# GBATZOLIS/conditional_score_diffusion

Measured on AMD Instinct MI355X. Metric: images/sec for 1000-step PC sampling, ddpm_paired_SR3 score net of celebA_SR3_160 (BASELINE configs[1]), 160x160, higher is better.
Workload: dtype f16x3 (every operand carried as hi + lo fp16 = 22 significand bits, 3 MFMAs per product, f32 accumulate; f32-class: the per-op test tolerance is the f32 kernel's, network error 1.9e-6 vs the reference); 1 GPU; BASELINE configs[1]: celebA_SR3_160 (ddpm_paired_SR3, nf=96, ch_mult (1,1,2,2,3,3), attn 20/10/5), 1000-step PC (reverse_diffusion + langevin, snr 0.15), batch 64 per GPU, random-init weights, synthetic LR inputs; images_per_gpu=64, global_batch=64, noise=on-device Philox4x32-10, precision_mode=fp16x3

## Files before the change

conditional_score_diffusion_amd/csrc/attention.hip:

```cpp
#include "common.h"

namespace csd {

typedef float floatx16 __attribute__((ext_vector_type(16)));

#define ATT_THREADS 256
#define ATT_KT 32

template <int NCT>
__global__ __launch_bounds__(ATT_THREADS) void attention_kernel(const float* __restrict__ qkv, int ld,
                                                                float* __restrict__ out, int L,
                                                                float scale) {
  constexpr int C = NCT * 32;
  constexpr int KS = C + 4;
  extern __shared__ __attribute__((aligned(16))) float smem[];
  float* const Ks = smem;
  float* const Vs = smem + ATT_KT * KS;

  const int tid = threadIdx.x;
  const int lane = tid & 63;
  const int wave = tid >> 6;
  const int half = lane >> 5;
  const int b = blockIdx.y;
  const int q0 = blockIdx.x * 128 + wave * 32;
  const bool wave_active = q0 < L;
  const int qrow = min(q0 + (lane & 31), L - 1);
  const float* qptr = qkv + ((size_t)b * L + qrow) * ld + half * 4;
  const float* kvbase = qkv + (size_t)b * L * ld;

  floatx16 o[NCT];
#pragma unroll
  for (int n = 0; n < NCT; ++n)
#pragma unroll
    for (int r = 0; r < 16; ++r) o[n][r] = 0.f;
  float m_run = -INFINITY;
  float l_run = 0.f;

  const int ntiles = (L + ATT_KT - 1) / ATT_KT;
  for (int t = 0; t < ntiles; ++t) {
    const int key0 = t * ATT_KT;
    __syncthreads();
    for (int e = tid; e < 2 * ATT_KT * (C / 4); e += ATT_THREADS) {
      const int which = e / (ATT_KT * (C / 4));
      const int r = e - which * ATT_KT * (C / 4);
      const int key = r / (C / 4);
      const int c4 = r - key * (C / 4);
      float4 v = make_float4(0.f, 0.f, 0.f, 0.f);
      if (key0 + key < L)
        v = *reinterpret_cast<const float4*>(kvbase + (size_t)(key0 + key) * ld + (1 + which) * C + c4 * 4);
      *reinterpret_cast<float4*>((which ? Vs : Ks) + key * KS + c4 * 4) = v;
    }
    __syncthreads();
    if (!wave_active) continue;

    floatx16 s;
#pragma unroll
    for (int r = 0; r < 16; ++r) s[r] = 0.f;
    const float* krow = Ks + (lane & 31) * KS + half * 4;
#pragma unroll 4
    for (int c0 = 0; c0 < C; c0 += 8) {
      const float4 a4 = *reinterpret_cast<const float4*>(krow + c0);
      const float4 b4 = *reinterpret_cast<const float4*>(qptr + c0);
      s = __builtin_amdgcn_mfma_f32_32x32x2f32(a4.x, b4.x, s, 0, 0, 0);
      s = __builtin_amdgcn_mfma_f32_32x32x2f32(a4.y, b4.y, s, 0, 0, 0);
      s = __builtin_amdgcn_mfma_f32_32x32x2f32(a4.z, b4.z, s, 0, 0, 0);
      s = __builtin_amdgcn_mfma_f32_32x32x2f32(a4.w, b4.w, s, 0, 0, 0);
    }
    float mt = -INFINITY;
#pragma unroll
    for (int r = 0; r < 16; ++r) {
      const int key = key0 + (r & 3) + 8 * (r >> 2) + 4 * half;
      s[r] = (key < L) ? s[r] * scale : -INFINITY;
      mt = fmaxf(mt, s[r]);
    }
    mt = fmaxf(mt, __shfl_xor(mt, 32));
    const float m_new = fmaxf(m_run, mt);
    const float alpha = expf(m_run - m_new);
    float psum = 0.f;
#pragma unroll
    for (int r = 0; r < 16; ++r) {
      s[r] = expf(s[r] - m_new);
      psum += s[r];
    }
    l_run = l_run * alpha + psum;
    m_run = m_new;
#pragma unroll
    for (int r = 0; r < 16; ++r) {
      const int row = (r & 3) + 8 * (r >> 2) + 4 * half;
      const float ar = __shfl(alpha, row);
#pragma unroll
      for (int n = 0; n < NCT; ++n) o[n][r] *= ar;
    }
#pragma unroll
    for (int r = 0; r < 16; ++r) {
      const float* vrow = Vs + ((r & 3) + 8 * (r >> 2) + 4 * half) * KS + (lane & 31);
#pragma unroll
      for (int n = 0; n < NCT; ++n)
        o[n] = __builtin_amdgcn_mfma_f32_32x32x2f32(s[r], vrow[n * 32], o[n], 0, 0, 0);
    }
  }

  if (!wave_active) return;
  const float l_tot = l_run + __shfl_xor(l_run, 32);
#pragma unroll
  for (int r = 0; r < 16; ++r) {
    const int row = (r & 3) + 8 * (r >> 2) + 4 * half;
    const float lr = __shfl(l_tot, row);
    const int q = q0 + row;
    if (q < L) {
      float* dst = out + ((size_t)b * L + q) * C + (lane & 31);
#pragma unroll
      for (int n = 0; n < NCT; ++n) dst[n * 32] = o[n][r] / lr;
    }
  }
}

template <int NCT>
static int launch_att(const float* qkv, int ld, float* out, int B, int L, hipStream_t s) {
  constexpr int C = NCT * 32;
  const size_t lds = (size_t)2 * ATT_KT * (C + 4) * sizeof(float);
  auto kern = attention_kernel<NCT>;
  static bool attr_set = false;
  if (!attr_set) {
    CSD_CHECK_HIP(hipFuncSetAttribute(reinterpret_cast<const void*>(kern),
                                      hipFuncAttributeMaxDynamicSharedMemorySize, 160 * 1024));
    attr_set = true;
  }
  const float scale = 1.0f / sqrtf((float)C);
  (void)scale;
  const float ref_scale = (float)pow((double)C, -0.5);
  hipLaunchKernelGGL(kern, dim3(cdiv(L, 128), B), dim3(ATT_THREADS), lds, s, qkv, ld, out, L, ref_scale);
  CSD_LAUNCH_CHECK();
  return CSD_OK;
}

typedef _Float16 half8a __attribute__((ext_vector_type(8)));
typedef _Float16 half4a __attribute__((ext_vector_type(4)));

template <int NCT, int NS, int CS>
__global__ __launch_bounds__(ATT_THREADS) void attention16_kernel(const float* __restrict__ qkv, int ld,
                                                                  float* __restrict__ out, int L, float scale) {
  constexpr int C = NCT * 32, KSTEPS = C / 16;
  constexpr int KS = 2 * C + 16;
  constexpr int VS = 80;
  constexpr int KPL = ATT_KT * KS, VPL = C * VS;
  extern __shared__ __attribute__((aligned(16))) char smem16[];
  char* const Kp = smem16;
  char* const Vp = smem16 + NS * KPL;

  const int tid = threadIdx.x;
  const int lane = tid & 63;
  const int wave = tid >> 6;
  const int kb = lane >> 5, l32 = lane & 31;
  const int b = blockIdx.y;
  constexpr int NOT = (NCT + CS - 1) / CS;
  const int n0 = (wave % CS) * NOT;
  const int q0 = blockIdx.x * (128 / CS) + (wave / CS) * 32;
  const bool wave_active = q0 < L;
  const float* kvbase = qkv + (size_t)b * L * ld;

  half8a qh[KSTEPS], ql[NS == 2 ? KSTEPS : 1];
  {
    const float* qptr = kvbase + (size_t)min(q0 + l32, L - 1) * ld + kb * 8;
#pragma unroll
    for (int ks = 0; ks < KSTEPS; ++ks) {
      const float4 a = *reinterpret_cast<const float4*>(qptr + ks * 16);
      const float4 c = *reinterpret_cast<const float4*>(qptr + ks * 16 + 4);
      const float v[8] = {a.x * scale, a.y * scale, a.z * scale, a.w * scale, c.x * scale, c.y * scale, c.z * scale, c.w * scale};
#pragma unroll
      for (int j = 0; j < 8; ++j) {
        const _Float16 h = (_Float16)v[j];
        qh[ks][j] = h;
        if (NS == 2) ql[ks][j] = (_Float16)(v[j] - (float)h);
      }
    }
  }

  floatx16 o[NOT];
#pragma unroll
  for (int n = 0; n < NOT; ++n)
#pragma unroll
    for (int r = 0; r < 16; ++r) o[n][r] = 0.f;
  float m_run = -INFINITY, l_run = 0.f;

  constexpr int NK = NCT;
  constexpr int NVG = (2 * C + ATT_THREADS - 1) / ATT_THREADS;
  float4 prek[NK], prev[NVG][4];
  auto prefetch = [&](int key0) {
#pragma unroll
    for (int i = 0; i < NK; ++i) {
      const int e = tid + i * ATT_THREADS;
      const int key = e / (C / 4), c4 = e - key * (C / 4);
      prek[i] = key0 + key < L ? *reinterpret_cast<const float4*>(kvbase + (size_t)(key0 + key) * ld + C + c4 * 4)
                               : make_float4(0.f, 0.f, 0.f, 0.f);
    }
#pragma unroll
    for (int i = 0; i < NVG; ++i) {
      const int g = tid + i * ATT_THREADS;
      const int m = g & 7, c4 = min(g >> 3, C / 4 - 1);
#pragma unroll
      for (int u = 0; u < 4; ++u) {
        const int key = key0 + 4 * m + u;
        prev[i][u] = key < L ? *reinterpret_cast<const float4*>(kvbase + (size_t)key * ld + 2 * C + c4 * 4)
                             : make_float4(0.f, 0.f, 0.f, 0.f);
      }
    }
  };
  auto commit = [&]() {
#pragma unroll
    for (int i = 0; i < NK; ++i) {
      const int e = tid + i * ATT_THREADS;
      const int key = e / (C / 4), c4 = e - key * (C / 4);
      const float v[4] = {prek[i].x, prek[i].y, prek[i].z, prek[i].w};
      half4a hi, lo;
#pragma unroll
      for (int j = 0; j < 4; ++j) {
        hi[j] = (_Float16)v[j];
        lo[j] = (_Float16)(v[j] - (float)hi[j]);
      }
      *reinterpret_cast<half4a*>(Kp + key * KS + c4 * 8) = hi;
      if (NS == 2) *reinterpret_cast<half4a*>(Kp + KPL + key * KS + c4 * 8) = lo;
    }
#pragma unroll
    for (int i = 0; i < NVG; ++i) {
      const int g = tid + i * ATT_THREADS;
      if (g >= 2 * C) continue;
      const int m = g & 7, c4 = g >> 3;
      const int w = (4 * m) & 15;
      const int pos = ((4 * m) & 16) + 8 * ((w >> 2) & 1) + 4 * (w >> 3);
#pragma unroll
      for (int j = 0; j < 4; ++j) {
        const float v[4] = {j == 0 ? prev[i][0].x : j == 1 ? prev[i][0].y : j == 2 ? prev[i][0].z : prev[i][0].w,
                            j == 0 ? prev[i][1].x : j == 1 ? prev[i][1].y : j == 2 ? prev[i][1].z : prev[i][1].w,
                            j == 0 ? prev[i][2].x : j == 1 ? prev[i][2].y : j == 2 ? prev[i][2].z : prev[i][2].w,
                            j == 0 ? prev[i][3].x : j == 1 ? prev[i][3].y : j == 2 ? prev[i][3].z : prev[i][3].w};
        half4a hi, lo;
#pragma unroll
        for (int u = 0; u < 4; ++u) {
          hi[u] = (_Float16)v[u];
          lo[u] = (_Float16)(v[u] - (float)hi[u]);
        }
        *reinterpret_cast<half4a*>(Vp + (c4 * 4 + j) * VS + pos * 2) = hi;
        if (NS == 2) *reinterpret_cast<half4a*>(Vp + VPL + (c4 * 4 + j) * VS + pos * 2) = lo;
      }
    }
  };

  constexpr bool AHEAD = NCT <= 6;
  const int ntiles = (L + ATT_KT - 1) / ATT_KT;
  if (AHEAD) prefetch(0);
  for (int t = 0; t < ntiles; ++t) {
    const int key0 = t * ATT_KT;
    if (!AHEAD) prefetch(key0);
    __syncthreads();
    commit();
    __syncthreads();
    if (AHEAD && t + 1 < ntiles) prefetch(key0 + ATT_KT);
    if (!wave_active) continue;

    floatx16 s;
#pragma unroll
    for (int r = 0; r < 16; ++r) s[r] = 0.f;
    const char* krow = Kp + l32 * KS + kb * 16;
    half8a ah_n = *reinterpret_cast<const half8a*>(krow), al_n;
    if (NS == 2) al_n = *reinterpret_cast<const half8a*>(krow + KPL);
#pragma unroll
    for (int ks = 0; ks < KSTEPS; ++ks) {
      const half8a ah = ah_n, al = al_n;
      if (ks + 1 < KSTEPS) {
        ah_n = *reinterpret_cast<const half8a*>(krow + (ks + 1) * 32);
        if (NS == 2) al_n = *reinterpret_cast<const half8a*>(krow + KPL + (ks + 1) * 32);
      }
      if (NS == 2) {
        s = __builtin_amdgcn_mfma_f32_32x32x16_f16(al, qh[ks], s, 0, 0, 0);
        s = __builtin_amdgcn_mfma_f32_32x32x16_f16(ah, ql[ks], s, 0, 0, 0);
      }
      s = __builtin_amdgcn_mfma_f32_32x32x16_f16(ah, qh[ks], s, 0, 0, 0);
      __builtin_amdgcn_sched_barrier(0);
    }
    float mt = -INFINITY;
#pragma unroll
    for (int r = 0; r < 16; ++r) {
      const int key = key0 + (r & 3) + 8 * (r >> 2) + 4 * kb;
      s[r] = (key < L) ? s[r] : -INFINITY;
      mt = fmaxf(mt, s[r]);
    }
    mt = fmaxf(mt, __shfl_xor(mt, 32));
    const float m_new = fmaxf(m_run, mt);
    const float alpha = __expf(m_run - m_new);
    float psum = 0.f;
    half8a ph[2], pl[NS == 2 ? 2 : 1];
#pragma unroll
    for (int r = 0; r < 16; ++r) {
      const float pv = __expf(s[r] - m_new);
      psum += pv;
      const _Float16 h = (_Float16)pv;
      ph[r >> 3][r & 7] = h;
      if (NS == 2) pl[r >> 3][r & 7] = (_Float16)(pv - (float)h);
    }
    l_run = l_run * alpha + psum;
    m_run = m_new;
    if (!__all(alpha == 1.0f)) {
#pragma unroll
      for (int r = 0; r < 16; ++r) {
        const float ar = __shfl(alpha, (r & 3) + 8 * (r >> 2) + 4 * kb);
#pragma unroll
        for (int n = 0; n < NOT; ++n) o[n][r] *= ar;
      }
    }
#pragma unroll
    for (int tt = 0; tt < 2; ++tt) {
      const char* vrow = Vp + (n0 * 32 + l32) * VS + (16 * tt + 8 * kb) * 2;
      half8a vh_n = *reinterpret_cast<const half8a*>(vrow), vl_n;
      if (NS == 2) vl_n = *reinterpret_cast<const half8a*>(vrow + VPL);
#pragma unroll
      for (int n = 0; n < NOT; ++n) {
        if (CS > 1 && n0 + n >= NCT) break;
        const half8a vh = vh_n, vl = vl_n;
        if (n + 1 < NOT && (CS == 1 || n0 + n + 1 < NCT)) {
          vh_n = *reinterpret_cast<const half8a*>(vrow + (n + 1) * 32 * VS);
          if (NS == 2) vl_n = *reinterpret_cast<const half8a*>(vrow + VPL + (n + 1) * 32 * VS);
        }
        if (NS == 2) {
          o[n] = __builtin_amdgcn_mfma_f32_32x32x16_f16(pl[tt], vh, o[n], 0, 0, 0);
          o[n] = __builtin_amdgcn_mfma_f32_32x32x16_f16(ph[tt], vl, o[n], 0, 0, 0);
        }
        o[n] = __builtin_amdgcn_mfma_f32_32x32x16_f16(ph[tt], vh, o[n], 0, 0, 0);
        __builtin_amdgcn_sched_barrier(0);
      }
    }
  }

  if (!wave_active) return;
  const float l_tot = l_run + __shfl_xor(l_run, 32);
#pragma unroll
  for (int r = 0; r < 16; ++r) {
    const int row = (r & 3) + 8 * (r >> 2) + 4 * kb;
    const float lr = __shfl(l_tot, row);
    const int q = q0 + row;
    if (q < L) {
      float* dst = out + ((size_t)b * L + q) * C + n0 * 32 + l32;
#pragma unroll
      for (int n = 0; n < NOT; ++n)
        if (CS == 1 || n0 + n < NCT) dst[n * 32] = o[n][r] / lr;
    }
  }
}

template <int NCT, int NS>
static int launch_att16(const float* qkv, int ld, float* out, int B, int L, hipStream_t s) {
  constexpr int C = NCT * 32;
  const size_t lds = (size_t)NS * (ATT_KT * (2 * C + 16) + C * 80);
  constexpr int CS = NCT >= 8 ? 2 : 1;
  auto kern = attention16_kernel<NCT, NS, CS>;
  static bool attr_set = false;
  if (!attr_set) {
    CSD_CHECK_HIP(hipFuncSetAttribute(reinterpret_cast<const void*>(kern),
                                      hipFuncAttributeMaxDynamicSharedMemorySize, 160 * 1024));
    attr_set = true;
  }
  const float ref_scale = (float)pow((double)C, -0.5);
  hipLaunchKernelGGL(kern, dim3(cdiv(L, 128 / CS), B), dim3(ATT_THREADS), lds, s, qkv, ld, out, L, ref_scale);
  CSD_LAUNCH_CHECK();
  return CSD_OK;
}

int attention16_launch(const float* qkv, int ld, float* out, int B, int L, int C, int ns, hipStream_t s) {
  CSD_REQUIRE(C % 32 == 0, "attention: C=%d must be a multiple of 32", C);
  CSD_REQUIRE(L >= 1, "attention: empty sequence");
  CSD_REQUIRE(ns == 1 || ns == 2, "attention16: %d operand planes", ns);
#define CSD_ATT16_CASE(N) case N: return ns == 2 ? launch_att16<N, 2>(qkv, ld, out, B, L, s) : launch_att16<N, 1>(qkv, ld, out, B, L, s);
  switch (C / 32) {
    CSD_ATT16_CASE(1) CSD_ATT16_CASE(2) CSD_ATT16_CASE(3) CSD_ATT16_CASE(4) CSD_ATT16_CASE(6) CSD_ATT16_CASE(8) CSD_ATT16_CASE(9)
    default:
      set_error("attention: C=%d not instantiated (supported: 32,64,96,128,192,256,288)", C);
      return CSD_ERR_INVALID;
  }
#undef CSD_ATT16_CASE
}

int attention_launch(const float* qkv, int ld, float* out, int B, int L, int C, hipStream_t s) {
  CSD_REQUIRE(C % 32 == 0, "attention: C=%d must be a multiple of 32", C);
  CSD_REQUIRE(L >= 1, "attention: empty sequence");
  switch (C / 32) {
    case 1: return launch_att<1>(qkv, ld, out, B, L, s);
    case 2: return launch_att<2>(qkv, ld, out, B, L, s);
    case 3: return launch_att<3>(qkv, ld, out, B, L, s);
    case 4: return launch_att<4>(qkv, ld, out, B, L, s);
    case 6: return launch_att<6>(qkv, ld, out, B, L, s);
    case 8: return launch_att<8>(qkv, ld, out, B, L, s);
    case 9: return launch_att<9>(qkv, ld, out, B, L, s);
    default:
      set_error("attention: C=%d not instantiated (supported: 32,64,96,128,192,256,288)", C);
      return CSD_ERR_INVALID;
  }
}

}
```

Measured before the change: 1.661 images/sec.

## Use buffer loads for K/V prefetch and pin attention accumulators in AGPRs

Replaces the per-element bounds-checked global loads of K and V tiles with raw buffer loads through a buffer resource whose range ends at row L, so out-of-range keys return zero from hardware instead of via per-load compares and 64-bit address math. Offsets are precomputed once as 32-bit values, and the wave index is made uniform with readfirstlane. For wide channel counts, the output accumulators are forced into accumulation registers via inline asm constraints, with the alpha rescale done through a VGPR round trip. This lowers VGPR pressure and address arithmetic, at the cost of a 4GB offset limit (now checked at launch) and possible extra moves between register files.

```diff
diff --git a/conditional_score_diffusion_amd/csrc/attention.hip b/conditional_score_diffusion_amd/csrc/attention.hip
--- a/conditional_score_diffusion_amd/csrc/attention.hip
+++ b/conditional_score_diffusion_amd/csrc/attention.hip
@@ -136,6 +136,8 @@
 
 typedef _Float16 half8a __attribute__((ext_vector_type(8)));
 typedef _Float16 half4a __attribute__((ext_vector_type(4)));
+typedef float att_f4 __attribute__((ext_vector_type(4)));
+#define ATT16_PAST 0x40000000u
 
 template <int NCT, int NS, int CS>
 __global__ __launch_bounds__(ATT_THREADS) void attention16_kernel(const float* __restrict__ qkv, int ld,
@@ -150,7 +152,7 @@
 
   const int tid = threadIdx.x;
   const int lane = tid & 63;
-  const int wave = tid >> 6;
+  const int wave = __builtin_amdgcn_readfirstlane(tid >> 6);
   const int kb = lane >> 5, l32 = lane & 31;
   const int b = blockIdx.y;
   constexpr int NOT = (NCT + CS - 1) / CS;
@@ -185,26 +187,28 @@
 
   constexpr int NK = NCT;
   constexpr int NVG = (2 * C + ATT_THREADS - 1) / ATT_THREADS;
-  float4 prek[NK], prev[NVG][4];
-  auto prefetch = [&](int key0) {
-#pragma unroll
-    for (int i = 0; i < NK; ++i) {
-      const int e = tid + i * ATT_THREADS;
-      const int key = e / (C / 4), c4 = e - key * (C / 4);
-      prek[i] = key0 + key < L ? *reinterpret_cast<const float4*>(kvbase + (size_t)(key0 + key) * ld + C + c4 * 4)
-                               : make_float4(0.f, 0.f, 0.f, 0.f);
-    }
-#pragma unroll
-    for (int i = 0; i < NVG; ++i) {
-      const int g = tid + i * ATT_THREADS;
-      const int m = g & 7, c4 = min(g >> 3, C / 4 - 1);
-#pragma unroll
-      for (int u = 0; u < 4; ++u) {
-        const int key = key0 + 4 * m + u;
-        prev[i][u] = key < L ? *reinterpret_cast<const float4*>(kvbase + (size_t)key * ld + 2 * C + c4 * 4)
-                             : make_float4(0.f, 0.f, 0.f, 0.f);
-      }
-    }
+  const unsigned ldb = (unsigned)ld * 4u;
+  unsigned kvo[NK];
+#pragma unroll
+  for (int i = 0; i < NK; ++i) {
+    const int e = tid + i * ATT_THREADS;
+    const int key = e / (C / 4), c4 = e - key * (C / 4);
+    kvo[i] = (unsigned)key * ldb + (unsigned)(C + c4 * 4) * 4u;
+  }
+  const unsigned vvo = (unsigned)(4 * (tid & 7)) * ldb + (unsigned)(2 * C + (tid >> 3) * 4) * 4u;
+  const unsigned vvo_last = tid + (NVG - 1) * ATT_THREADS < 2 * C ? vvo + (NVG - 1) * 512u : ATT16_PAST;
+  att_f4 prek[NK], prev[NVG][4];
+  auto prefetch = [&](int key0) __attribute__((always_inline)) {
+    const __amdgpu_buffer_rsrc_t rows = __builtin_amdgcn_make_buffer_rsrc(const_cast<float*>(kvbase + (size_t)key0 * ld), 0,
+                                                                          (unsigned)(L - key0) * ldb, 0x00020000);
+#pragma unroll
+    for (int i = 0; i < NK; ++i) prek[i] = __builtin_bit_cast(att_f4, __builtin_amdgcn_raw_buffer_load_b128(rows, kvo[i], 0, 0));
+#pragma unroll
+    for (int i = 0; i < NVG; ++i)
+#pragma unroll
+      for (int u = 0; u < 4; ++u)
+        prev[i][u] = __builtin_bit_cast(
+            att_f4, __builtin_amdgcn_raw_buffer_load_b128(rows, (i == NVG - 1 ? vvo_last : vvo + i * 512u) + u * ldb, 0, 0));
   };
   auto commit = [&]() {
 #pragma unroll
@@ -300,13 +304,24 @@
     }
     l_run = l_run * alpha + psum;
     m_run = m_new;
+    constexpr bool O_IN_ACC = NCT >= 6;
     if (!__all(alpha == 1.0f)) {
-#pragma unroll
-      for (int r = 0; r < 16; ++r) {
-        const float ar = __shfl(alpha, (r & 3) + 8 * (r >> 2) + 4 * kb);
-#pragma unroll
-        for (int n = 0; n < NOT; ++n) o[n][r] *= ar;
-      }
+      float ar[16];
+#pragma unroll
+      for (int r = 0; r < 16; ++r) ar[r] = __shfl(alpha, (r & 3) + 8 * (r >> 2) + 4 * kb);
+#pragma unroll
+      for (int n = 0; n < NOT; ++n) {
+        floatx16 v = o[n];
+        if (O_IN_ACC) asm volatile("" : "+v"(v));
+#pragma unroll
+        for (int r = 0; r < 16; ++r) v[r] *= ar[r];
+        if (O_IN_ACC) asm volatile("" : "+a"(v));
+        o[n] = v;
+      }
+    }
+    if (O_IN_ACC) {
+#pragma unroll
+      for (int n = 0; n < NOT; ++n) asm volatile("" : "+a"(o[n]));
     }
 #pragma unroll
     for (int tt = 0; tt < 2; ++tt) {
@@ -352,6 +367,7 @@
   constexpr int C = NCT * 32;
   const size_t lds = (size_t)NS * (ATT_KT * (2 * C + 16) + C * 80);
   constexpr int CS = NCT >= 8 ? 2 : 1;
+  CSD_REQUIRE((size_t)L * ld * 4 < ATT16_PAST,"attention16: L=%d rows of %d floats exceed the K / V descriptor range", L, ld);
   auto kern = attention16_kernel<NCT, NS, CS>;
   static bool attr_set = false;
   if (!attr_set) {
```

Measured after the change: 1.669 images/sec, median of 6. No clear change (+0.5%).
